# dfyz/osm-renderer

Hardware: AMD Instinct MI355X
Metric: tiles/sec (256x256 z=15) (higher is better)
Workload: dtype f64; 1 GPU; BASELINE.json configs[1]: batch of 1024 z=15 256x256 tiles per GPU, synthetic 50-poly/200-segment geometry per tile (SplitMix64, SURVEY.md 8(d)), lat/lon f64 input resident in HBM, RGBA8 framebuffers written to HBM; 2 batches in flight (step i on resident copy / stream i mod 2: the pre-pass of one batch overlaps the raster stage of the previous one); tiles_this_rank=1024, polygons_per_tile=50, polylines_per_tile=40, scale=1, named_config=True, collective=none (1 GPU), rccl_nranks_seen=1, batches_in_flight=2

## Files before the change

osm_renderer_amd/build.py:

```python
import os
import shutil
import subprocess

HERE = os.path.dirname(os.path.abspath(__file__))
CSRC = os.path.join(HERE, "csrc")
LIB = os.path.join(HERE, "libosmtile.so")
SOURCES = ["osmt_kernels.hip", "osmt_labels.hip", "osmt_glyphs.hip", "osmt_textplace.hip", "osmt_textshape.hip", "osmt_polylabel.hip", "osmt_styled.hip", "osmt_tilequery.hip", "osmt_tilelabels.hip", "osmt_arealabels.hip", "osmt_selmatch.hip", "osmt_labelbind.hip", "osmt_cascade.hip", "osmt_anchors.hip", "osmt_pngenc.hip", "osmt_api.cpp", "osmt_png.cpp"]
HEADERS = ["osmt_bitonic.h", "osmt_cascade_rule.h", "osmt_cascade_tables.h", "osmt_fill_slots.h", "osmt_geom.h", "osmt_glyph.h", "osmt_internal.h", "osmt_list_slices.h", "osmt_numparse.h", "osmt_png_table.h", "osmt_prebin_roles.h", "osmt_project.h", "osmt_utf8.h", os.path.join("..", "host", "osmt_textplacer.hpp"),
           os.path.join("..", "host", "osmt_textshaper.hpp"),
           os.path.join("..", "..", "include", "osmtile.h")]
LIBS = ["-lz", "-ldl", "-lpthread", "-Wl,--no-undefined"]
FLAGS = ["--offload-arch=gfx950", "-O3", "-std=c++17", "-ffp-contract=off", "-fPIC", "-shared", "-Wall"]


def _hipcc():
    for cand in (shutil.which("hipcc"), "/opt/rocm/bin/hipcc"):
        if cand and os.path.exists(cand):
            return cand
    raise RuntimeError("hipcc not found; libosmtile.so cannot be built")


def needs_build():
    if not os.path.exists(LIB):
        return True
    t = os.path.getmtime(LIB)
    deps = [os.path.join(CSRC, s) for s in SOURCES + HEADERS]
    return any(os.path.getmtime(d) > t for d in deps)


def build_variant(name, defines):
    out = os.path.join(HERE, f"libosmtile_{name}.so")
    cmd = [_hipcc()] + FLAGS + [f"-D{d}" for d in defines] + ["-o", out] + [os.path.join(CSRC, s) for s in SOURCES] + LIBS
    subprocess.check_call(cmd)
    return out


def build(force=False, verbose=False):
    if not force and not needs_build():
        return LIB
    cmd = [_hipcc()] + FLAGS + ["-o", LIB] + [os.path.join(CSRC, s) for s in SOURCES] + LIBS
    if verbose:
# ... 8 lines not shown
```

osm_renderer_amd/csrc/osmt_kernels.hip:

```cpp
#include <hip/hip_runtime.h>
#include <stdint.h>

#include "../../include/osmtile.h"
#include "osmt_geom.h"
#include "osmt_internal.h"
#include "osmt_prebin_roles.h"
#include "osmt_project.h"

namespace {

__device__ __forceinline__ uint32_t f64_as_u8(double v) {
#if defined(__HIP_DEVICE_COMPILE__) && !defined(OSMT_V_PLAIN_CVT)
    uint32_t r;
    asm("v_cvt_u32_f64 %0, %1" : "=v"(r) : "v"(v));
    return min(r, 255u);
#else
    return (uint32_t)(int32_t)fmin(fmax(v, 0.0), 255.0);
#endif
}

__device__ __forceinline__ uint32_t wave_incl_scan(uint32_t x) {
    x += (uint32_t)__builtin_amdgcn_update_dpp(0, (int)x, 0x111, 0xF, 0xF, false);
    x += (uint32_t)__builtin_amdgcn_update_dpp(0, (int)x, 0x112, 0xF, 0xF, false);
    x += (uint32_t)__builtin_amdgcn_update_dpp(0, (int)x, 0x114, 0xF, 0xF, false);
    x += (uint32_t)__builtin_amdgcn_update_dpp(0, (int)x, 0x118, 0xF, 0xF, false);
    x += (uint32_t)__builtin_amdgcn_update_dpp(0, (int)x, 0x142, 0xA, 0xF, false);
    x += (uint32_t)__builtin_amdgcn_update_dpp(0, (int)x, 0x143, 0xC, 0xF, false);
    return x;
}

__global__ __launch_bounds__(256) void k_project(const osmt_tile_job* __restrict__ jobs,
                                                 const uint32_t* __restrict__ pt_job,
                                                 const double2* __restrict__ latlon, const uint32_t* __restrict__ refs,
                                                 uint32_t n_pts, double scale, int2* __restrict__ pts, uint32_t* __restrict__ zero,
                                                 uint32_t n_zero) {
    const uint32_t i = blockIdx.x * 256u + threadIdx.x;
    if (i < n_zero) zero[i] = 0u;
    if (i >= n_pts) return;
    const uint32_t j = pt_job[i];
    if (j == 0xFFFFFFFFu) {
// ... 378 lines not shown
            const uint32_t first = q_base + osmt_fill_slot_first(0u, q_incl, nsr);
            const uint32_t g = oi.fill_geom;
            bool past = false;
            for (uint32_t r = 0; r < nsr; ++r) {
                if ((unsigned long long)first + r >= a.slot_cap) {
                    past = true;
                    break;
                }
                a.slots[first + r] = g ? osmt_fill_slot_make(o, oi.arena_off, r, g & 255u, (g >> 8) & 255u, (g >> 16) & 255u, oi.n_rings,
                                                             oi.n_edges, oi.first_pt)
                                       : osmt_fill_slot_empty();
            }
            if (past && a.err) *(volatile uint32_t*)a.err = OSMT_PREPASS_ERR_FILL_ARENA;
        }
    }
    if (live) a.info[o] = oi;
}

__device__ __forceinline__ double opacity_by_center_distance(double cd, double hlw) {
    const double feather_from = fmax(hlw - 0.5, 0.0);
    const double feather_to = fmax(hlw + 0.5, 1.0);
    const double feather_dist = feather_to - feather_from;
    const double opacity_mul = fmin(2.0 * hlw, 1.0);
    double v;
    if (cd < feather_from)
        v = 1.0;
    else if (cd < feather_to)
        v = (feather_to - cd) / feather_dist;
    else
        v = 0.0;
    return opacity_mul * v;
}

#define OSMT_C4(i) (double)(i) / 255.0, (double)((i) + 1) / 255.0, (double)((i) + 2) / 255.0, (double)((i) + 3) / 255.0
#define OSMT_C16(i) OSMT_C4(i), OSMT_C4((i) + 4), OSMT_C4((i) + 8), OSMT_C4((i) + 12)
#define OSMT_C64(i) OSMT_C16(i), OSMT_C16((i) + 16), OSMT_C16((i) + 32), OSMT_C16((i) + 48)
__constant__ double k_u8_over_255[256] = {OSMT_C64(0), OSMT_C64(64), OSMT_C64(128), OSMT_C64(192)};

constexpr int SUB = OSMT_SUB_W;
constexpr int SUBH = OSMT_SUB_H;
constexpr int NTHREADS = 64;
constexpr int PXT = SUB * SUBH / NTHREADS;
constexpr int ROWSTEP = NTHREADS / SUB;
#ifndef OSMT_V_OPCHUNK
#define OSMT_V_OPCHUNK 16
#endif
constexpr int OPCHUNK = OSMT_V_OPCHUNK;
static_assert(OPCHUNK == 16 || OPCHUNK == 32 || OPCHUNK == 64, "a chunk is staged by one wave");
#ifndef OSMT_V_SEGCAP
#define OSMT_V_SEGCAP 32
#endif
constexpr int SEGCAP = OSMT_V_SEGCAP;
static_assert(SEGCAP >= 8 && SEGCAP <= 64, "a filter pass is at most one wave wide");
#ifndef OSMT_V_PLANE_STRIDE
#define OSMT_V_PLANE_STRIDE 32
#endif
constexpr int PLANE_STRIDE = OSMT_V_PLANE_STRIDE;

#if defined(OSMT_ABL) && OSMT_ABL == 5
#define OSMT_DBG(...) __VA_ARGS__
#else
#define OSMT_DBG(...)
#endif
struct alignas(16) StagedEnt {
    double c0, c1, c2;
    double op;
    uint32_t arena;
    uint32_t kind_stage;
    uint32_t aux;
    uint32_t nv;
};
static_assert(sizeof(StagedEnt) == 48, "three 16-byte LDS loads");
struct StrokeConst {
    double ff0, ft0, fd0, rfd0, mul0;
    uint32_t flags;
    uint32_t _pad;
};
constexpr uint32_t STROKE_PLAIN_MAIN = 1u;
constexpr uint32_t STROKE_UNIT_FD = 2u;
constexpr uint32_t STROKE_TINY_MUL = 4u;
constexpr uint32_t STROKE_DASH_FAST = 8u;
__device__ __forceinline__ uint32_t stroke_flags(const osmt_stroke_aux* __restrict__ sa) {
    const bool tiny = !(sa->mul0 >= 1e-100);
    const int n = sa->main_n_segs;
#ifdef OSMT_V_NO_DASH_FAST
    const bool fast = false;
#else
    const bool fast = n > 0 && sa->main_has_orig == 0 && sa->main_total_len > 0.0 && !tiny;
#endif
    return (n == 0 ? STROKE_PLAIN_MAIN : 0u) | (sa->fd0 == 1.0 ? STROKE_UNIT_FD : 0u) | (tiny ? STROKE_TINY_MUL : 0u) | (fast ? STROKE_DASH_FAST : 0u);
}
#ifndef OSMT_V_STAGECAP
#define OSMT_V_STAGECAP 16
#endif
constexpr int STAGECAP = OSMT_V_STAGECAP;

struct alignas(8) SegDer {
    int32_t a, b;
    float r2b, r2a;
    uint32_t w;
    uint32_t n_main;
    double ru, rv;
};
static_assert(sizeof(SegDer) == 40, "five 8-byte LDS words");
constexpr uint32_t SEGW_INCX_NEG = 1u, SEGW_INCY_NEG = 2u, SEGW_SWAP = 4u, SEGW_CAP = 8u, SEGW_SLOW = 16u;

#ifndef OSMT_V_FILTCAP
#define OSMT_V_FILTCAP 256
#endif
constexpr uint32_t FILTCAP = OSMT_V_FILTCAP;
#if OSMT_V_OPCHUNK <= OSMT_V_STAGECAP
#define OSMT_STAGE_UNION 1
#else
#define OSMT_STAGE_UNION 0
#endif
constexpr int DTAB_F = 7;
struct RasterShared {
    OSMT_DBG(uint32_t dbg[12];)
    osmt_srec seg[SEGCAP];
    SegDer der[SEGCAP];
    uint32_t pre[SEGCAP];
    unsigned long long plane[PLANE_STRIDE * SUBH];
    StagedEnt ent[OPCHUNK];
    uint32_t nvi[OPCHUNK];
#if OSMT_STAGE_UNION
    union {
        uint32_t fmask[SUBH];
        StrokeConst sconst;
    } stg[STAGECAP];
#else
    uint32_t fmask_[STAGECAP][SUBH];
    StrokeConst sconst_[STAGECAP];
#endif
    double dtab[OSMT_MAX_DASH_SEGS][DTAB_F];
    uint32_t queue[64];
#ifdef OSMT_V_LDSPAD
    uint8_t occupancy_experiment_pad[OSMT_V_LDSPAD];
#endif
};
#if !(defined(OSMT_ABL) && OSMT_ABL == 5)
static_assert(sizeof(RasterShared) <= 10240, "16 waves per CU (four per SIMD) share 160 KB of LDS");
#endif
#if OSMT_STAGE_UNION
#define SH_FMASK(sh, st) ((sh).stg[st].fmask)
#define SH_SCONST(sh, st) ((sh).stg[st].sconst)
#else
#define SH_FMASK(sh, st) ((sh).fmask_[st])
#define SH_SCONST(sh, st) ((sh).sconst_[st])
// ... 353 lines not shown
                        if (kind == 1u) {
                            const double num = ft0 - cd;
                            const double qv = fd0 == 1.0 ? num : osmt_div_exact(num, fd0, rfd0);
                            const double cdop = mul0 * (cd < ff0 ? 1.0 : qv);
                            atomicMax(&sh.plane[st.ry * PLANE_STRIDE + st.rx], (unsigned long long)__double_as_longlong(initial_opacity * cdop));
                        }
                    } else {
                        slow = true;
                    }
                }
            }
            const unsigned long long sb = __ballot(slow);
            if (sb) {
                const uint32_t ns = (uint32_t)__popcll(sb);
                if (qn + ns > 64u) {
                    dashed_drain(sh, qn, kc, n, total, r_total, initial_opacity, rc);
                    qn = 0u;
                }
                if (slow) sh.queue[qn + (uint32_t)__popcll(sb & ((1ull << fresh_lane()) - 1ull))] = slot_tag | ((uint32_t)st.ry << 5) | (uint32_t)st.rx;
                qn += ns;
            }
            if (active) {
                const bool corr = st.err + st.two_a > st.b;
                dotv += corr ? dot_step + dot_corr : dot_step;
                walk_advance(st);
            }
        }
    }
    if (qn) dashed_drain(sh, qn, kc, n, total, r_total, initial_opacity, rc);
}

template <class Shared>
__device__ __forceinline__ void walk_items(Shared& sh, uint32_t lane, uint32_t slot0, uint32_t nslot, uint32_t item_base, uint32_t it_lo, uint32_t it_hi,
                                           const StrokeConst& kc, uint32_t sflags, const osmt_stroke_aux* __restrict__ sa, double initial_opacity,
                                           const SubRect& rc) {
    OSMT_DBG(if (lane == 0u) { sh.dbg[1] += (it_hi - it_lo + 63u) / 64u; sh.dbg[2] += it_hi - it_lo; })
    const bool main_plain = (sflags & STROKE_PLAIN_MAIN) != 0u;
    const bool unit_fd = (sflags & (STROKE_UNIT_FD | STROKE_TINY_MUL)) == STROKE_UNIT_FD;
    const bool dash_fast = (sflags & STROKE_DASH_FAST) != 0u;
    if (dash_fast) {
        walk_items_dashed(sh, slot0, nslot, item_base, it_lo, it_hi, kc, sa->main_n_segs, sa->main_total_len, sa->main_r_total, initial_opacity, rc);
        const uint32_t l_ = fresh_lane();
        if (!__ballot(l_ < nslot && (sh.der[slot0 + l_].w & SEGW_CAP) != 0u)) return;
    }
    for (uint32_t it = it_lo + lane; it < it_hi; it += 64u) {
        uint32_t lo_s = slot0, n = nslot;
        while (n > 1u) {
            const uint32_t half = n >> 1;
            const bool right = sh.pre[lo_s + half - 1u] <= it;
            lo_s = right ? lo_s + half : lo_s;
            n = right ? n - half : half;
        }
        const uint32_t base_items = (lo_s == slot0) ? item_base : sh.pre[lo_s - 1u];
        const osmt_srec& r = sh.seg[lo_s];
        const SegDer& d = sh.der[lo_s];
        const bool is_cap = (d.w & SEGW_CAP) != 0u;
        RunState st;
        bool skip_first;
        walk_setup(st, r, d, it - base_items, rc, &skip_first);
        if (main_plain && !is_cap) {
            if (unit_fd)
                walk_plain<true>(st, kc, initial_opacity, skip_first, sh.plane);
            else
                walk_plain<false>(st, kc, initial_opacity, skip_first, sh.plane);
        } else {
#ifndef OSMT_V_NODASH
#pragma unroll 1
            for (uint32_t t = main_plain ? 1u : 0u; t < 2u; ++t) {
                if (is_cap != (t == 1u)) continue;
                if (dash_fast && t == 0u) continue;
#ifdef OSMT_V_SKIPHEAVY
                if (t == (OSMT_V_SKIPHEAVY - 1)) continue;
#endif
                const bool cp = t == 1u;
                const osmt_raster_args* la = late_args();
                const osmt_dash_seg* sgs = cp ? &sa->caps_seg : la->dseg + (size_t)(sa - la->aux) * OSMT_MAX_DASH_SEGS;
                walk_dashed(st, kc, cp ? 1 : sa->main_n_segs, (cp ? sa->caps_has_orig : sa->main_has_orig) != 0, cp ? 0.0 : sa->main_total_len,
                            cp ? 0.0 : sa->main_r_total, sgs, sa->half_width, r.traveled, initial_opacity, sh.plane);
            }
#endif
        }
    }
}

__device__ __noinline__ uint32_t fill_row_streaming(const osmt_ring* __restrict__ rings, const int2* __restrict__ pts,
                                                    uint32_t ring_off, uint32_t n_rings, int32_t y, int32_t x0,
                                                    int32_t x1) {
    uint32_t m = 0u;
    int32_t last_x = INT32_MIN;
    int64_t last_e = -1;
    bool have_last = false;
    uint32_t k = 0;
    int32_t from_x = 0;
    for (;;) {
        bool found = false;
        int32_t bx = 0, bxm = 0;
        int64_t be = 0;
        uint32_t eb = 0;
        for (uint32_t r = 0; r < n_rings; ++r) {
            const osmt_ring ring = rings[ring_off + r];
            if (ring.n_pts < 2) continue;
            for (uint32_t e = 0; e + 1 < ring.n_pts; ++e) {
                const int2 p1 = pts[ring.first_pt + e];
                const int2 p2 = pts[ring.first_pt + e + 1];
                int32_t xmn, xmx;
                if (!osmt_fill_row_extent(p1.x, p1.y, p2.x, p2.y, y, &xmn, &xmx)) continue;
                const int64_t ge = (int64_t)eb + e;
                const bool after = !have_last || xmn > last_x || (xmn == last_x && ge > last_e);
                if (!after) continue;
                if (!found || xmn < bx || (xmn == bx && ge < be)) {
                    found = true;
// ... 649 lines not shown
#else
    unsigned long long save;
    double t0, t1, t2, k;
    asm volatile(
        "v_cmp_lt_f64 vcc, 0, %[al]\n\t"
        "s_and_saveexec_b64 %[sv], vcc\n\t"
        "s_cbranch_execz 1f\n\t"
        "v_mul_f64 %[t0], %[al], %[c0]\n\t"
        "v_mul_f64 %[t1], %[al], %[c1]\n\t"
        "v_mul_f64 %[t2], %[al], %[c2]\n\t"
        "v_add_f64 %[k], 1.0, -%[al]\n\t"
        "v_mul_f64 %[r], %[k], %[r]\n\t"
        "v_mul_f64 %[g], %[k], %[g]\n\t"
        "v_mul_f64 %[b], %[k], %[b]\n\t"
        "v_add_f64 %[r], %[t0], %[r]\n\t"
        "v_add_f64 %[g], %[t1], %[g]\n\t"
        "v_add_f64 %[b], %[t2], %[b]\n"
        "1:\n\t"
        "s_mov_b64 exec, %[sv]"
        : [r] "+v"(r), [g] "+v"(g), [b] "+v"(b), [sv] "=&s"(save), [t0] "=&v"(t0), [t1] "=&v"(t1), [t2] "=&v"(t2), [k] "=&v"(k)
        : [al] "v"(al), [c0] "v"(c0), [c1] "v"(c1), [c2] "v"(c2)
        : "vcc", "scc");
#endif
}

template <bool OUT_F64, bool LABELS, bool FOLD>
__global__ OSMT_RASTER_BOUNDS void k_raster(
    const osmt_raster_args a) {
    const osmt_ent* OSMT_R g_ent = a.ent;
    const osmt_stroke_aux* OSMT_R g_aux = a.aux;
    const uint32_t* OSMT_R g_fmask = a.fmask;
    const osmt_srec* OSMT_R g_srec = a.srec;
    const uint2* OSMT_R g_skey = a.skey;
    const uint32_t g_scale = a.scale;
    __shared__ RasterShared sh;

    const uint32_t tid = threadIdx.x;
    const uint32_t lane = tid;
    const uint32_t W = OSMT_TILE_SIZE * g_scale;
    const uint32_t subs_per_row = W / SUB;
    const uint32_t nsub = subs_per_row * (W / SUBH);

    const uint32_t b = blockIdx.x;
    const uint32_t xcd = b & 7u;
    const uint32_t rest = b >> 3;
    const uint32_t tile = (rest / nsub) * 8u + xcd;
    const uint32_t sub = rest % nsub;
    if (tile >= a.n_jobs) return;

    const osmt_tile_job job = a.jobs[tile];
    SubRect rc;
    const uint32_t sub_x = sub % subs_per_row, sub_y = sub / subs_per_row;
    rc.x0 = (int32_t)(sub_x * SUB);
    rc.y0 = (int32_t)(sub_y * SUBH);
    rc.x1 = rc.x0 + SUB - 1;
    rc.y1 = rc.y0 + SUBH - 1;


#ifdef OSMT_V_ACCPROBE
#define AJ(j) ((j) % OSMT_V_ACCPROBE)
#else
#define AJ(j) (j)
#endif
    double acc[PXT][3];
    {
        double r = 0.0, g = 0.0, bl = 0.0;
        if (job.has_canvas) {
            r = 1.0 * k_u8_over_255[job.canvas_rgb[0]];
            g = 1.0 * k_u8_over_255[job.canvas_rgb[1]];
            bl = 1.0 * k_u8_over_255[job.canvas_rgb[2]];
        }
#pragma unroll
        for (int j = 0; j < PXT; ++j) {
            acc[AJ(j)][0] = r;
            acc[AJ(j)][1] = g;
            acc[AJ(j)][2] = bl;
        }
    }
    bool plane_clean = false;
    OSMT_DBG(if (lane < 12) sh.dbg[lane] = 0u; __syncthreads();)

    const bool fold = FOLD && job.n_ops <= OSMT_FOLD_MAX_OPS;
    auto op_bits = [&](unsigned long long* b0, unsigned long long* b1) {
        const osmt_raster_args* la = late_args();
        const osmt_tile_job* OSMT_R jb = &la->jobs[tile];
        const uint32_t n_ops = jb->n_ops, sub_rows = W / SUBH;
        const uint32_t* OSMT_R sm = la->submask + (size_t)jb->op_off * sub_rows + sub / subs_per_row;
        const uint32_t t_ = fresh_lane(), sx_ = sub % subs_per_row;
        const uint32_t w0 = t_ < n_ops ? sm[(size_t)t_ * sub_rows] : 0u;
        const uint32_t w1 = t_ + 64u < n_ops ? sm[(size_t)(t_ + 64u) * sub_rows] : 0u;
        *b0 = __ballot((w0 >> sx_) & 1u);
        *b1 = __ballot((w1 >> sx_) & 1u);
    };
    uint2 hdr = make_uint2(0u, 0u);
    if (fold) {
        unsigned long long b0, b1;
        op_bits(&b0, &b1);
        hdr.y = (uint32_t)__popcll(b0) + (uint32_t)__popcll(b1);
    } else {
        hdr = a.hdr[(size_t)tile * nsub + sub];
        if (job.n_ops == 0u) hdr = make_uint2(0u, 0u);
    }
#if defined(OSMT_ABL) && OSMT_ABL == 8
    const uint32_t n_ent = hdr.y > 0xFFFFFFF0u ? 1u : 0u;
#else
    const uint32_t n_ent = hdr.y;
#endif
    const osmt_ent* OSMT_R my_ent = g_ent + hdr.x;

    for (uint32_t base = 0; base < n_ent; base += OPCHUNK) {
        const uint32_t total = min((uint32_t)OPCHUNK, n_ent - base);
        const bool hit = lane < total;
        osmt_ent e = {};
        if (FOLD && late_args()->jobs[tile].n_ops <= OSMT_FOLD_MAX_OPS) {
            osmt_ent* const tmp = reinterpret_cast<osmt_ent*>(sh.seg);
            static_assert(sizeof(osmt_ent) * OPCHUNK <= sizeof(sh.seg), "a chunk's entries fit the record array");
            const osmt_opinfo* OSMT_R g_info = late_args()->info + late_args()->jobs[tile].op_off;
            unsigned long long bb[2];
            op_bits(&bb[0], &bb[1]);
            const uint32_t n0 = (uint32_t)__popcll(bb[0]);
#pragma unroll
            for (uint32_t half = 0; half < 2u; ++half) {
                const uint32_t t_ = fresh_lane();
                const uint32_t r = (half ? n0 : 0u) + (uint32_t)__popcll(bb[half] & ((1ull << t_) - 1ull));
                if (((bb[half] >> t_) & 1ull) && r >= base && r < base + (uint32_t)OPCHUNK) {
                    const osmt_opinfo* OSMT_R hi = &g_info[t_ + 64u * half];
                    const uint32_t kind = hi->kind;
                    const bool strk = kind == OSMT_OP_STROKE;
                    const uint32_t geom = hi->fill_geom, arena0 = hi->arena_off;
                    osmt_ent t;
                    t.kind_color = kind | ((uint32_t)hi->color[0] << 8) | ((uint32_t)hi->color[1] << 16) | ((uint32_t)hi->color[2] << 24);
                    t.opacity = hi->opacity;
                    t.aux = strk ? hi->aux : hi->image_id;
                    t.nv = strk ? hi->rec_cap : 0u;
                    t.arena = strk ? arena0
                                   : (arena0 + (sub / subs_per_row - (geom & 255u)) * ((geom >> 16) & 255u) + (sub % subs_per_row - ((geom >> 8) & 255u))) * SUBH;
                    t.stage = 0u;
                    t._pad = 0u;
                    tmp[r - base] = t;
                }
            }
            __syncthreads();
            if (hit) e = tmp[fresh_lane()];
        } else if (hit) {
            e = my_ent[base + lane];
        }
        const uint32_t e_kind = e.kind_color & 255u;
        const bool is_stroke = hit && e_kind == OSMT_OP_STROKE;
        const unsigned long long sbal = __ballot(is_stroke);
#if OSMT_STAGE_UNION
        const uint32_t my_stage = fresh_lane();
#else
        const unsigned long long fbal = __ballot(hit && !is_stroke);
        const uint32_t my_stage = (uint32_t)__popcll((is_stroke ? sbal : fbal) & ((1ull << fresh_lane()) - 1ull));
#endif
        const uint32_t nv_scan = wave_incl_scan(is_stroke ? min(e.nv, 1u << 20) : 0u);
        __syncthreads();
        if (hit) {
            sh.nvi[fresh_lane()] = nv_scan;
            StagedEnt se;
            const double cr = k_u8_over_255[(e.kind_color >> 8) & 255u], cg = k_u8_over_255[(e.kind_color >> 16) & 255u],
                         cb = k_u8_over_255[e.kind_color >> 24];
            const bool fc = e_kind == OSMT_OP_FILL_COLOR;
            se.c0 = fc ? e.opacity * cr : cr;
            se.c1 = fc ? e.opacity * cg : cg;
            se.c2 = fc ? e.opacity * cb : cb;
            se.op = fc ? 1.0 - e.opacity : e.opacity;
            se.arena = e.arena;
            se.kind_stage = e_kind | ((my_stage < (uint32_t)STAGECAP ? my_stage : 255u) << 8);
            se.aux = e.aux;
            se.nv = e.nv;
            sh.ent[lane] = se;
            if (!is_stroke && my_stage < (uint32_t)STAGECAP) {
                const uint4* OSMT_R src = reinterpret_cast<const uint4*>(g_fmask + e.arena);
                uint4* dst = reinterpret_cast<uint4*>(&SH_FMASK(sh, my_stage)[0]);
                const uint4 w0 = src[0], w1 = src[1], w2 = src[2], w3 = src[3];
                dst[0] = w0;
                dst[1] = w1;
                dst[2] = w2;
                dst[3] = w3;
            }
            if (is_stroke && my_stage < (uint32_t)STAGECAP) {
                const osmt_stroke_aux* __restrict__ sa = &g_aux[e.aux];
                StrokeConst kc;
                kc.ff0 = sa->ff0;
                kc.ft0 = sa->ft0;
                kc.fd0 = sa->fd0;
                kc.rfd0 = sa->rfd0;
                kc.mul0 = sa->mul0;
                kc.flags = stroke_flags(sa);
                kc._pad = 0;
                SH_SCONST(sh, my_stage) = kc;
            }
        }
        const bool any_stroke = sbal != 0ull;
        if (any_stroke && !plane_clean) {
            static_assert((PLANE_STRIDE * SUBH) % NTHREADS == 0, "the plane is cleared in whole wave strides");
            const uint32_t t_ = fresh_lane();
#pragma unroll
            for (uint32_t i = 0; i < PLANE_STRIDE * SUBH; i += NTHREADS) sh.plane[i + t_] = 0ull;
            plane_clean = true;
        }
        __syncthreads();

        uint32_t g0 = 0;
#if defined(OSMT_ABL) && OSMT_ABL == 7
        if (total < 1000u) g0 = total;
#endif
        while (g0 < total) {
        uint32_t gend = total, V = 0;
        bool big = false;
        uint32_t s_before = 0u;
        const uint32_t nv_incl = any_stroke ? sh.nvi[fresh_lane() & (uint32_t)(OPCHUNK - 1)] : 0u;
        if (any_stroke) {
            s_before = g0 ? (uint32_t)__builtin_amdgcn_readlane((int)nv_incl, (int)g0 - 1) : 0u;
            const unsigned long long over = __ballot(lane >= g0 && lane < total && nv_incl - s_before > (uint32_t)FILTCAP);
            if (over) gend = (uint32_t)__builtin_ctzll(over);
            if (gend == g0) {
                OSMT_DBG(if (lane == 0) sh.dbg[7] += 1u;)
                big = true;
                gend = g0 + 1u;
            } else {
                V = (uint32_t)__builtin_amdgcn_readlane((int)nv_incl, (int)gend - 1) - s_before;
            }
        }
        if (V) {
// ... 109 lines not shown
            }
            __syncthreads();
        }
        unsigned long long gbal = 0ull;

        for (uint32_t li = g0; li < gend; ++li) {
            const StagedEnt& en = sh.ent[li];
            const uint32_t ks = (uint32_t)__builtin_amdgcn_readfirstlane((int)en.kind_stage);
            const uint32_t kind = ks & 255u, stage = ks >> 8;
            const double cop = en.op;
#if defined(OSMT_ABL) && OSMT_ABL == 6
            if (kind != 77u) continue;
#endif
#if defined(OSMT_ABL) && OSMT_ABL == 3
            if (kind == OSMT_OP_STROKE) continue;
#endif
#if defined(OSMT_ABL) && OSMT_ABL == 4
            if (kind != OSMT_OP_STROKE) continue;
#endif
            if (kind == OSMT_OP_STROKE) {
                OSMT_DBG(if (lane == 0) sh.dbg[0] += 1u;)
                const uint32_t aux_i = (uint32_t)__builtin_amdgcn_readfirstlane((int)en.aux);
                const osmt_stroke_aux* __restrict__ sa = &g_aux[aux_i];
                StrokeConst kc;
                if (stage != 255u) {
                    kc = SH_SCONST(sh, stage);
                } else {
                    kc.ff0 = sa->ff0;
                    kc.ft0 = sa->ft0;
                    kc.fd0 = sa->fd0;
                    kc.rfd0 = sa->rfd0;
                    kc.mul0 = sa->mul0;
                    kc.flags = stroke_flags(sa);
                    kc._pad = 0;
                }
                const uint32_t sflags = (uint32_t)__builtin_amdgcn_readfirstlane((int)kc.flags);
                if (sflags & STROKE_DASH_FAST) {
                    const double* OSMT_R src = reinterpret_cast<const double*>(late_args()->dseg + (size_t)aux_i * OSMT_MAX_DASH_SEGS);
                    static_assert(sizeof(osmt_dash_seg) == 9 * sizeof(double), "nine doubles per DashSegment");
                    const uint32_t nd = (uint32_t)sa->main_n_segs * (uint32_t)DTAB_F;
                    for (uint32_t l = fresh_lane(); l < nd; l += 64u) {
                        const uint32_t sg = l / (uint32_t)DTAB_F, f = l % (uint32_t)DTAB_F;
                        (&sh.dtab[0][0])[l] = src[sg * 9u + (f < 5u ? f : f + 2u)];
                    }
                    __syncthreads();
                }
                uint32_t n_rounds = 1u, big_cap = 0u, arena = 0u;
                if (big) {
                    big_cap = (uint32_t)__builtin_amdgcn_readfirstlane((int)en.nv);
                    arena = (uint32_t)__builtin_amdgcn_readfirstlane((int)en.arena);
                    n_rounds = (big_cap + (uint32_t)SEGCAP - 1u) / (uint32_t)SEGCAP;
                }
                for (uint32_t round = 0; round < n_rounds; ++round) {
                    uint32_t slot0 = 0u, nslot = 0u;
                    if (big) {
                        __syncthreads();
                        uint32_t ridx = 0xFFFFFFFFu;
                        const uint32_t v = round * (uint32_t)SEGCAP + lane;
                        if (lane < (uint32_t)SEGCAP && v < big_cap) ridx = arena + v;
                        uint32_t cnt = 0, is_cap = 0;
                        if (ridx != 0xFFFFFFFFu) {
                            const uint2 key = g_skey[ridx];
                            if (key.x == sub) {
                                cnt = key.y & 0x7FFFFFFFu;
                                is_cap = key.y >> 31;
                            }
                        }
                        gbal = __ballot(cnt > 0u);
                        const uint32_t incl = wave_incl_scan(cnt);
                        if (cnt > 0u) {
                            const uint32_t slot = (uint32_t)__popcll(gbal & ((1ull << fresh_lane()) - 1ull));
                            const osmt_srec r = g_srec[ridx];
                            sh.seg[slot] = r;
                            sh.der[slot] = seg_derive(r, is_cap != 0u);
                            sh.pre[slot] = incl;
                        }
                        __syncthreads();
                        nslot = (uint32_t)__popcll(gbal);
                    } else {
                        slot0 = (uint32_t)__builtin_amdgcn_readfirstlane((int)en.arena);
                        nslot = (uint32_t)__builtin_amdgcn_readfirstlane((int)en.nv);
                    }
                    {
                        if (nslot) {
                            const uint32_t item_lo = slot0 ? (uint32_t)__builtin_amdgcn_readfirstlane((int)sh.pre[slot0 - 1u]) : 0u;
                            const uint32_t item_hi = (uint32_t)__builtin_amdgcn_readfirstlane((int)sh.pre[slot0 + nslot - 1u]);
#if defined(OSMT_ABL) && (OSMT_ABL == 1 || OSMT_ABL == 2)
                            (void)item_lo; (void)item_hi;
#else
                            walk_items(sh, lane, slot0, nslot, item_lo, item_lo, item_hi, kc, sflags, sa, cop, rc);
#endif
                        }
                    }
                }
                __syncthreads();
#if defined(OSMT_ABL) && OSMT_ABL == 2
                if (false)
#endif
                {
                    const StagedEnt& eb = sh.ent[late_index(li)];
                    const double c0 = eb.c0, c1 = eb.c1, c2 = eb.c2;
                    const uint32_t t_ = fresh_lane();
                    const uint32_t cell0 = (t_ / SUB) * PLANE_STRIDE + (t_ & (SUB - 1));
#pragma unroll
                    for (int j = 0; j < PXT; ++j) {
                        const uint32_t idx = cell0 + (uint32_t)j * ROWSTEP * PLANE_STRIDE;
                        const double al = __longlong_as_double((long long)sh.plane[idx]);
                        sh.plane[idx] = 0ull;
                        blend_stroke_masked(acc[AJ(j)][0], acc[AJ(j)][1], acc[AJ(j)][2], al, c0, c1, c2);
                    }
                }
                __syncthreads();
            }
            if (late_index(kind) != OSMT_OP_STROKE) {
                OSMT_DBG(if (lane == 0) sh.dbg[5] += 1u;)
                uint32_t w_[SUBH];
                if (stage != 255u) {
                    const uint4* OSMT_R lw = reinterpret_cast<const uint4*>(&SH_FMASK(sh, stage)[0]);
#pragma unroll
                    for (int q = 0; q < SUBH / 4; ++q) {
                        const uint4 v = lw[q];
                        w_[4 * q + 0] = v.x;
                        w_[4 * q + 1] = v.y;
// ... 95 lines not shown
            }
          }
        }
    }

    void* const g_out = late_args()->out;
    const size_t g_out_tile_stride = late_args()->out_tile_stride;
    const uint32_t t_out = fresh_lane();
    const uint32_t lx_o = t_out & (SUB - 1), ly_o = t_out / SUB;
    if (!OUT_F64 && late_args()->out_rgb8) {
        uint8_t* const stg = reinterpret_cast<uint8_t*>(sh.plane);
        static_assert(sizeof(sh.plane) >= (size_t)SUB * SUBH * 3, "RGB8 staging fits the alpha plane");
        __syncthreads();
#pragma unroll
        for (int j = 0; j < PXT; ++j) {
            const uint32_t row = ly_o + (uint32_t)j * ROWSTEP;
            uint8_t* px = stg + (row * SUB + lx_o) * 3u;
            px[0] = (uint8_t)f64_as_u8(255.0 * acc[AJ(j)][0]);
            px[1] = (uint8_t)f64_as_u8(255.0 * acc[AJ(j)][1]);
            px[2] = (uint8_t)f64_as_u8(255.0 * acc[AJ(j)][2]);
        }
        __syncthreads();
        constexpr uint32_t ROW_DW = SUB * 3 / 4;
        uint8_t* const tile_out = reinterpret_cast<uint8_t*>(g_out) + (size_t)tile * g_out_tile_stride;
#pragma unroll
        for (uint32_t q = 0; q < ROW_DW * SUBH / NTHREADS; ++q) {
            const uint32_t d = q * NTHREADS + t_out;
            const uint32_t row = d / ROW_DW, k = d % ROW_DW;
            const uint32_t v = reinterpret_cast<const uint32_t*>(stg)[d];
            __builtin_nontemporal_store(v, reinterpret_cast<uint32_t*>(tile_out + ((size_t)(rc.y0 + (int32_t)row) * W + (size_t)rc.x0) * 3u + 4u * k));
        }
        return;
    }
#pragma unroll
    for (int j = 0; j < PXT; ++j) {
        const uint32_t row = ly_o + (uint32_t)j * ROWSTEP;
        const size_t px = (size_t)(rc.y0 + (int32_t)row) * W + (size_t)(rc.x0 + (int32_t)lx_o);
        if (OUT_F64) {
            double4* out = reinterpret_cast<double4*>(g_out) + (size_t)tile * W * W + px;
            *out = make_double4(acc[AJ(j)][0], acc[AJ(j)][1], acc[AJ(j)][2], 1.0);
        } else {
            const uint32_t v = f64_as_u8(255.0 * acc[AJ(j)][0]) | (f64_as_u8(255.0 * acc[AJ(j)][1]) << 8) |
                               (f64_as_u8(255.0 * acc[AJ(j)][2]) << 16) | 0xFF000000u;
            uint32_t* out = reinterpret_cast<uint32_t*>(reinterpret_cast<uint8_t*>(g_out) +
                                                        (size_t)tile * g_out_tile_stride) + px;
#ifdef OSMT_V_PLAIN_STORE
            *out = v;
#else
            __builtin_nontemporal_store(v, out);
#endif
            OSMT_DBG(__syncthreads(); if (j == 0 && ly_o == 0 && lx_o < 12) *out = sh.dbg[lx_o];)
        }
    }
}

typedef double v2d __attribute__((ext_vector_type(2)));

__device__ __forceinline__ double dpp_swap_pair(double x) {
    const long long b = __double_as_longlong(x);
    const int lo = __builtin_amdgcn_update_dpp(0, (int)(b & 0xFFFFFFFFll), 0xB1, 0xF, 0xF, false);
    const int hi = __builtin_amdgcn_update_dpp(0, (int)(b >> 32), 0xB1, 0xF, 0xF, false);
    return __longlong_as_double(((long long)hi << 32) | (unsigned int)lo);
}

template <int LT, bool NT>
__global__ __launch_bounds__(256) void k_composite(const v2d* __restrict__ planes, double4 canvas, uint32_t n,
// ... 201 lines not shown
```

Before: 1.488 million tiles/s.

## Shorten raster kernel dependency chains at start, staging, dash visit and store

Several small latency-chain reductions in the raster kernel. Job and header records are now loaded with explicit scalar loads, and the canvas colour is computed arithmetically instead of through a constant-memory table lookup. Entry staging issues the fill-mask and stroke-aux loads early as vector words and builds the stroke constants from them, with the dash main-segment fields cached in LDS so walk_items no longer reads global aux. The RGBA8 store path uses precomputed byte offsets. Each piece is gated by a macro; the inline asm and layout static_asserts add fragility.

New measurement: 1.553 million tiles/s (median of 6 runs). 4.3% higher.

```diff
diff --git a/osm_renderer_amd/build.py b/osm_renderer_amd/build.py
--- a/osm_renderer_amd/build.py
+++ b/osm_renderer_amd/build.py
@@ -6,7 +6,7 @@
 CSRC = os.path.join(HERE, "csrc")
 LIB = os.path.join(HERE, "libosmtile.so")
 SOURCES = ["osmt_kernels.hip", "osmt_labels.hip", "osmt_glyphs.hip", "osmt_textplace.hip", "osmt_textshape.hip", "osmt_polylabel.hip", "osmt_styled.hip", "osmt_tilequery.hip", "osmt_tilelabels.hip", "osmt_arealabels.hip", "osmt_selmatch.hip", "osmt_labelbind.hip", "osmt_cascade.hip", "osmt_anchors.hip", "osmt_pngenc.hip", "osmt_api.cpp", "osmt_png.cpp"]
-HEADERS = ["osmt_bitonic.h", "osmt_cascade_rule.h", "osmt_cascade_tables.h", "osmt_fill_slots.h", "osmt_geom.h", "osmt_glyph.h", "osmt_internal.h", "osmt_list_slices.h", "osmt_numparse.h", "osmt_png_table.h", "osmt_prebin_roles.h", "osmt_project.h", "osmt_utf8.h", os.path.join("..", "host", "osmt_textplacer.hpp"),
+HEADERS = ["osmt_bitonic.h", "osmt_cascade_rule.h", "osmt_cascade_tables.h", "osmt_fill_slots.h", "osmt_geom.h", "osmt_glyph.h", "osmt_internal.h", "osmt_list_slices.h", "osmt_numparse.h", "osmt_png_table.h", "osmt_prebin_roles.h", "osmt_project.h", "osmt_u8_over_255.h", "osmt_utf8.h", os.path.join("..", "host", "osmt_textplacer.hpp"),
            os.path.join("..", "host", "osmt_textshaper.hpp"),
            os.path.join("..", "..", "include", "osmtile.h")]
 LIBS = ["-lz", "-ldl", "-lpthread", "-Wl,--no-undefined"]
diff --git a/osm_renderer_amd/csrc/osmt_kernels.hip b/osm_renderer_amd/csrc/osmt_kernels.hip
--- a/osm_renderer_amd/csrc/osmt_kernels.hip
+++ b/osm_renderer_amd/csrc/osmt_kernels.hip
@@ -6,6 +6,7 @@
 #include "osmt_internal.h"
 #include "osmt_prebin_roles.h"
 #include "osmt_project.h"
+#include "osmt_u8_over_255.h"
 
 namespace {
 
@@ -450,19 +451,39 @@
     return opacity_mul * v;
 }
 
-#define OSMT_C4(i) (double)(i) / 255.0, (double)((i) + 1) / 255.0, (double)((i) + 2) / 255.0, (double)((i) + 3) / 255.0
-#define OSMT_C16(i) OSMT_C4(i), OSMT_C4((i) + 4), OSMT_C4((i) + 8), OSMT_C4((i) + 12)
-#define OSMT_C64(i) OSMT_C16(i), OSMT_C16((i) + 16), OSMT_C16((i) + 32), OSMT_C16((i) + 48)
-__constant__ double k_u8_over_255[256] = {OSMT_C64(0), OSMT_C64(64), OSMT_C64(128), OSMT_C64(192)};
 
 constexpr int SUB = OSMT_SUB_W;
 constexpr int SUBH = OSMT_SUB_H;
 constexpr int NTHREADS = 64;
 constexpr int PXT = SUB * SUBH / NTHREADS;
 constexpr int ROWSTEP = NTHREADS / SUB;
+#ifndef OSMT_V_CHAIN_START
+#define OSMT_V_CHAIN_START 1
+#endif
+#ifndef OSMT_V_CHAIN_COLOR
+#define OSMT_V_CHAIN_COLOR 1
+#endif
+#ifndef OSMT_V_CHAIN_STAGE
+#define OSMT_V_CHAIN_STAGE 1
+#endif
+#ifndef OSMT_V_CHAIN_VISIT
+#define OSMT_V_CHAIN_VISIT 1
+#endif
+#ifndef OSMT_V_CHAIN_STORE
+#define OSMT_V_CHAIN_STORE 1
+#endif
 #ifndef OSMT_V_OPCHUNK
 #define OSMT_V_OPCHUNK 16
 #endif
+#ifndef OSMT_V_STAGECAP
+#define OSMT_V_STAGECAP 16
+#endif
+#if OSMT_V_OPCHUNK <= OSMT_V_STAGECAP
+#define OSMT_STAGE_UNION 1
+#else
+#define OSMT_STAGE_UNION 0
+#endif
+#define OSMT_CHAIN_VISIT (OSMT_V_CHAIN_VISIT && OSMT_STAGE_UNION)
 constexpr int OPCHUNK = OSMT_V_OPCHUNK;
 static_assert(OPCHUNK == 16 || OPCHUNK == 32 || OPCHUNK == 64, "a chunk is staged by one wave");
 #ifndef OSMT_V_SEGCAP
@@ -492,8 +513,18 @@
 struct StrokeConst {
     double ff0, ft0, fd0, rfd0, mul0;
     uint32_t flags;
+#if OSMT_CHAIN_VISIT
+    uint32_t n_segs;
+    double total_len, r_total;
+#else
     uint32_t _pad;
+#endif
 };
+#if OSMT_CHAIN_VISIT
+#define OSMT_KC_MAIN(sh, stage, sa, f, m) (SH_SCONST(sh, late_index(stage)).f)
+#else
+#define OSMT_KC_MAIN(sh, stage, sa, f, m) ((sa)->m)
+#endif
 constexpr uint32_t STROKE_PLAIN_MAIN = 1u;
 constexpr uint32_t STROKE_UNIT_FD = 2u;
 constexpr uint32_t STROKE_TINY_MUL = 4u;
@@ -508,9 +539,6 @@
 #endif
     return (n == 0 ? STROKE_PLAIN_MAIN : 0u) | (sa->fd0 == 1.0 ? STROKE_UNIT_FD : 0u) | (tiny ? STROKE_TINY_MUL : 0u) | (fast ? STROKE_DASH_FAST : 0u);
 }
-#ifndef OSMT_V_STAGECAP
-#define OSMT_V_STAGECAP 16
-#endif
 constexpr int STAGECAP = OSMT_V_STAGECAP;
 
 struct alignas(8) SegDer {
@@ -527,11 +555,6 @@
 #define OSMT_V_FILTCAP 256
 #endif
 constexpr uint32_t FILTCAP = OSMT_V_FILTCAP;
-#if OSMT_V_OPCHUNK <= OSMT_V_STAGECAP
-#define OSMT_STAGE_UNION 1
-#else
-#define OSMT_STAGE_UNION 0
-#endif
 constexpr int DTAB_F = 7;
 struct RasterShared {
     OSMT_DBG(uint32_t dbg[12];)
@@ -951,14 +974,15 @@
 
 template <class Shared>
 __device__ __forceinline__ void walk_items(Shared& sh, uint32_t lane, uint32_t slot0, uint32_t nslot, uint32_t item_base, uint32_t it_lo, uint32_t it_hi,
-                                           const StrokeConst& kc, uint32_t sflags, const osmt_stroke_aux* __restrict__ sa, double initial_opacity,
-                                           const SubRect& rc) {
+                                           const StrokeConst& kc, uint32_t stage, uint32_t sflags, const osmt_stroke_aux* __restrict__ sa,
+                                           double initial_opacity, const SubRect& rc) {
     OSMT_DBG(if (lane == 0u) { sh.dbg[1] += (it_hi - it_lo + 63u) / 64u; sh.dbg[2] += it_hi - it_lo; })
     const bool main_plain = (sflags & STROKE_PLAIN_MAIN) != 0u;
     const bool unit_fd = (sflags & (STROKE_UNIT_FD | STROKE_TINY_MUL)) == STROKE_UNIT_FD;
     const bool dash_fast = (sflags & STROKE_DASH_FAST) != 0u;
     if (dash_fast) {
-        walk_items_dashed(sh, slot0, nslot, item_base, it_lo, it_hi, kc, sa->main_n_segs, sa->main_total_len, sa->main_r_total, initial_opacity, rc);
+        walk_items_dashed(sh, slot0, nslot, item_base, it_lo, it_hi, kc, OSMT_KC_MAIN(sh, stage, sa, n_segs, main_n_segs), OSMT_KC_MAIN(sh, stage, sa, total_len, main_total_len),
+                          OSMT_KC_MAIN(sh, stage, sa, r_total, main_r_total), initial_opacity, rc);
         const uint32_t l_ = fresh_lane();
         if (!__ballot(l_ < nslot && (sh.der[slot0 + l_].w & SEGW_CAP) != 0u)) return;
     }
@@ -994,8 +1018,8 @@
                 const bool cp = t == 1u;
                 const osmt_raster_args* la = late_args();
                 const osmt_dash_seg* sgs = cp ? &sa->caps_seg : la->dseg + (size_t)(sa - la->aux) * OSMT_MAX_DASH_SEGS;
-                walk_dashed(st, kc, cp ? 1 : sa->main_n_segs, (cp ? sa->caps_has_orig : sa->main_has_orig) != 0, cp ? 0.0 : sa->main_total_len,
-                            cp ? 0.0 : sa->main_r_total, sgs, sa->half_width, r.traveled, initial_opacity, sh.plane);
+                walk_dashed(st, kc, cp ? 1 : (int)OSMT_KC_MAIN(sh, stage, sa, n_segs, main_n_segs), (cp ? sa->caps_has_orig : sa->main_has_orig) != 0,
+                            cp ? 0.0 : OSMT_KC_MAIN(sh, stage, sa, total_len, main_total_len), cp ? 0.0 : OSMT_KC_MAIN(sh, stage, sa, r_total, main_r_total), sgs, sa->half_width, r.traveled, initial_opacity, sh.plane);
             }
 #endif
         }
@@ -1711,7 +1735,15 @@
     const uint32_t* OSMT_R g_fmask = a.fmask;
     const osmt_srec* OSMT_R g_srec = a.srec;
     const uint2* OSMT_R g_skey = a.skey;
+#if OSMT_V_CHAIN_START
+    const osmt_tile_job* OSMT_R g_jobs = a.jobs;
+    const uint2* OSMT_R g_hdr = a.hdr;
+    uint32_t g_n_jobs = a.n_jobs;
+    uint32_t g_scale = a.scale;
+    asm("" : "+s"(g_n_jobs), "+s"(g_scale) : "s"(g_jobs), "s"(g_hdr), "s"(g_ent), "s"(g_aux), "s"(g_fmask), "s"(g_srec), "s"(g_skey));
+#else
     const uint32_t g_scale = a.scale;
+#endif
     __shared__ RasterShared sh;
 
     const uint32_t tid = threadIdx.x;
@@ -1725,9 +1757,39 @@
     const uint32_t rest = b >> 3;
     const uint32_t tile = (rest / nsub) * 8u + xcd;
     const uint32_t sub = rest % nsub;
+#if OSMT_V_CHAIN_START
+    if (tile >= g_n_jobs) return;
+
+    struct alignas(32) JobWords {
+        uint32_t w[8];
+    };
+    static_assert(sizeof(osmt_tile_job) == sizeof(JobWords) && offsetof(osmt_tile_job, has_canvas) == 9 && offsetof(osmt_tile_job, canvas_rgb) == 10 &&
+                      offsetof(osmt_tile_job, n_ops) == 16 && offsetof(osmt_tile_job, op_off) == 20,
+                  "the job record as words");
+    uint32_t job_w2, job_w3, job_n_ops;
+    uint2 hdr_raw = make_uint2(0u, 0u);
+    if (FOLD) {
+        const JobWords jw = *reinterpret_cast<const JobWords*>(g_jobs + tile);
+        job_w2 = jw.w[2], job_w3 = jw.w[3], job_n_ops = jw.w[4];
+    } else {
+        typedef uint32_t u32x4 __attribute__((ext_vector_type(4)));
+        typedef uint32_t u32x2 __attribute__((ext_vector_type(2)));
+        u32x4 jq;
+        u32x2 hq;
+        asm("s_load_dwordx4 %0, %2, 0x8\n\t"
+            "s_load_dwordx2 %1, %3, 0x0\n\t"
+            "s_waitcnt lgkmcnt(0)"
+            : "=&s"(jq), "=&s"(hq)
+            : "s"(g_jobs + tile), "s"(g_hdr + ((size_t)tile * nsub + sub)));
+        job_w2 = jq.x, job_w3 = jq.y, job_n_ops = jq.z;
+        hdr_raw = make_uint2(hq.x, hq.y);
+    }
+#else
     if (tile >= a.n_jobs) return;
 
     const osmt_tile_job job = a.jobs[tile];
+    const uint32_t job_n_ops = job.n_ops;
+#endif
     SubRect rc;
     const uint32_t sub_x = sub % subs_per_row, sub_y = sub / subs_per_row;
     rc.x0 = (int32_t)(sub_x * SUB);
@@ -1744,11 +1806,24 @@
     double acc[PXT][3];
     {
         double r = 0.0, g = 0.0, bl = 0.0;
+#if OSMT_V_CHAIN_START
+        const bool has_canvas = ((job_w2 >> 8) & 255u) != 0u;
+        auto uniform = [](double v) {
+            const long long b = __double_as_longlong(v);
+            const uint32_t lo = (uint32_t)__builtin_amdgcn_readfirstlane((int)(b & 0xFFFFFFFFll));
+            const uint32_t hi = (uint32_t)__builtin_amdgcn_readfirstlane((int)(b >> 32));
+            return __longlong_as_double((long long)(((unsigned long long)hi << 32) | lo));
+        };
+        r = uniform(osmt_u8_over_255(has_canvas ? (job_w2 >> 16) & 255u : 0u));
+        g = uniform(osmt_u8_over_255(has_canvas ? job_w2 >> 24 : 0u));
+        bl = uniform(osmt_u8_over_255(has_canvas ? job_w3 & 255u : 0u));
+#else
         if (job.has_canvas) {
             r = 1.0 * k_u8_over_255[job.canvas_rgb[0]];
             g = 1.0 * k_u8_over_255[job.canvas_rgb[1]];
             bl = 1.0 * k_u8_over_255[job.canvas_rgb[2]];
         }
+#endif
 #pragma unroll
         for (int j = 0; j < PXT; ++j) {
             acc[AJ(j)][0] = r;
@@ -1759,7 +1834,7 @@
     bool plane_clean = false;
     OSMT_DBG(if (lane < 12) sh.dbg[lane] = 0u; __syncthreads();)
 
-    const bool fold = FOLD && job.n_ops <= OSMT_FOLD_MAX_OPS;
+    const bool fold = FOLD && job_n_ops <= OSMT_FOLD_MAX_OPS;
     auto op_bits = [&](unsigned long long* b0, unsigned long long* b1) {
         const osmt_raster_args* la = late_args();
         const osmt_tile_job* OSMT_R jb = &la->jobs[tile];
@@ -1777,8 +1852,12 @@
         op_bits(&b0, &b1);
         hdr.y = (uint32_t)__popcll(b0) + (uint32_t)__popcll(b1);
     } else {
+#if OSMT_V_CHAIN_START
+        hdr = FOLD ? a.hdr[(size_t)tile * nsub + sub] : hdr_raw;
+#else
         hdr = a.hdr[(size_t)tile * nsub + sub];
-        if (job.n_ops == 0u) hdr = make_uint2(0u, 0u);
+#endif
+        if (job_n_ops == 0u) hdr = make_uint2(0u, 0u);
     }
 #if defined(OSMT_ABL) && OSMT_ABL == 8
     const uint32_t n_ent = hdr.y > 0xFFFFFFF0u ? 1u : 0u;
@@ -1837,9 +1916,18 @@
         __syncthreads();
         if (hit) {
             sh.nvi[fresh_lane()] = nv_scan;
+#if OSMT_V_CHAIN_STAGE && OSMT_STAGE_UNION
+            const uint4* OSMT_R src = is_stroke ? reinterpret_cast<const uint4*>(&g_aux[e.aux]) + 1 : reinterpret_cast<const uint4*>(g_fmask + e.arena);
+            const uint4 w0 = src[0], w1 = src[1], w2 = src[2], w3 = src[3];
+#endif
             StagedEnt se;
+#if OSMT_V_CHAIN_COLOR
+            const double cr = osmt_u8_over_255((e.kind_color >> 8) & 255u), cg = osmt_u8_over_255((e.kind_color >> 16) & 255u),
+                         cb = osmt_u8_over_255(e.kind_color >> 24);
+#else
             const double cr = k_u8_over_255[(e.kind_color >> 8) & 255u], cg = k_u8_over_255[(e.kind_color >> 16) & 255u],
                          cb = k_u8_over_255[e.kind_color >> 24];
+#endif
             const bool fc = e_kind == OSMT_OP_FILL_COLOR;
             se.c0 = fc ? e.opacity * cr : cr;
             se.c1 = fc ? e.opacity * cg : cg;
@@ -1850,6 +1938,42 @@
             se.aux = e.aux;
             se.nv = e.nv;
             sh.ent[lane] = se;
+#if OSMT_V_CHAIN_STAGE && OSMT_STAGE_UNION
+            {
+                static_assert(offsetof(osmt_stroke_aux, ff0) == 16 && offsetof(osmt_stroke_aux, ft0) == 24 && offsetof(osmt_stroke_aux, fd0) == 32 &&
+                                  offsetof(osmt_stroke_aux, mul0) == 40 && offsetof(osmt_stroke_aux, rfd0) == 48 &&
+                                  offsetof(osmt_stroke_aux, main_n_segs) == 56 && offsetof(osmt_stroke_aux, main_has_orig) == 60 &&
+                                  offsetof(osmt_stroke_aux, main_total_len) == 64 && offsetof(osmt_stroke_aux, main_r_total) == 72 &&
+                                  sizeof(StrokeConst) == (OSMT_CHAIN_VISIT ? 64 : 48) && sizeof(uint32_t) * SUBH == 64,
+                              "the words the stroke constants are put together from");
+                uint4* dst = reinterpret_cast<uint4*>(&SH_FMASK(sh, my_stage)[0]);
+                dst[0] = w0;
+                if (is_stroke) {
+                    auto f64_of = [](uint32_t lo, uint32_t hi) { return __longlong_as_double((long long)(((unsigned long long)hi << 32) | lo)); };
+                    const double fd0 = f64_of(w1.x, w1.y), mul0 = f64_of(w1.z, w1.w), total_len = f64_of(w3.x, w3.y);
+                    const int n = (int)w2.z;
+                    const bool tiny = !(mul0 >= 1e-100);
+#ifdef OSMT_V_NO_DASH_FAST
+                    const bool fast = false;
+#else
+                    const bool fast = n > 0 && w2.w == 0u && total_len > 0.0 && !tiny;
+#endif
+                    const uint32_t flags =
+                        (n == 0 ? STROKE_PLAIN_MAIN : 0u) | (fd0 == 1.0 ? STROKE_UNIT_FD : 0u) | (tiny ? STROKE_TINY_MUL : 0u) | (fast ? STROKE_DASH_FAST : 0u);
+                    dst[1] = make_uint4(w1.x, w1.y, w2.x, w2.y);
+#if OSMT_CHAIN_VISIT
+                    dst[2] = make_uint4(w1.z, w1.w, flags, w2.z);
+                    dst[3] = w3;
+#else
+                    dst[2] = make_uint4(w1.z, w1.w, flags, 0u);
+#endif
+                } else {
+                    dst[1] = w1;
+                    dst[2] = w2;
+                    dst[3] = w3;
+                }
+            }
+#else
             if (!is_stroke && my_stage < (uint32_t)STAGECAP) {
                 const uint4* OSMT_R src = reinterpret_cast<const uint4*>(g_fmask + e.arena);
                 uint4* dst = reinterpret_cast<uint4*>(&SH_FMASK(sh, my_stage)[0]);
@@ -1868,9 +1992,16 @@
                 kc.rfd0 = sa->rfd0;
                 kc.mul0 = sa->mul0;
                 kc.flags = stroke_flags(sa);
+#if OSMT_CHAIN_VISIT
+                kc.n_segs = (uint32_t)sa->main_n_segs;
+                kc.total_len = sa->main_total_len;
+                kc.r_total = sa->main_r_total;
+#else
                 kc._pad = 0;
+#endif
                 SH_SCONST(sh, my_stage) = kc;
             }
+#endif
         }
         const bool any_stroke = sbal != 0ull;
         if (any_stroke && !plane_clean) {
@@ -2046,13 +2177,19 @@
                     kc.rfd0 = sa->rfd0;
                     kc.mul0 = sa->mul0;
                     kc.flags = stroke_flags(sa);
+#if OSMT_CHAIN_VISIT
+                    kc.n_segs = (uint32_t)sa->main_n_segs;
+                    kc.total_len = sa->main_total_len;
+                    kc.r_total = sa->main_r_total;
+#else
                     kc._pad = 0;
+#endif
                 }
                 const uint32_t sflags = (uint32_t)__builtin_amdgcn_readfirstlane((int)kc.flags);
                 if (sflags & STROKE_DASH_FAST) {
                     const double* OSMT_R src = reinterpret_cast<const double*>(late_args()->dseg + (size_t)aux_i * OSMT_MAX_DASH_SEGS);
                     static_assert(sizeof(osmt_dash_seg) == 9 * sizeof(double), "nine doubles per DashSegment");
-                    const uint32_t nd = (uint32_t)sa->main_n_segs * (uint32_t)DTAB_F;
+                    const uint32_t nd = (uint32_t)OSMT_KC_MAIN(sh, stage, sa, n_segs, main_n_segs) * (uint32_t)DTAB_F;
                     for (uint32_t l = fresh_lane(); l < nd; l += 64u) {
                         const uint32_t sg = l / (uint32_t)DTAB_F, f = l % (uint32_t)DTAB_F;
                         (&sh.dtab[0][0])[l] = src[sg * 9u + (f < 5u ? f : f + 2u)];
@@ -2102,7 +2239,7 @@
 #if defined(OSMT_ABL) && (OSMT_ABL == 1 || OSMT_ABL == 2)
                             (void)item_lo; (void)item_hi;
 #else
-                            walk_items(sh, lane, slot0, nslot, item_lo, item_lo, item_hi, kc, sflags, sa, cop, rc);
+                            walk_items(sh, lane, slot0, nslot, item_lo, item_lo, item_hi, kc, stage, sflags, sa, cop, rc);
 #endif
                         }
                     }
@@ -2264,6 +2401,20 @@
         }
         return;
     }
+#if OSMT_V_CHAIN_STORE
+    if (!OUT_F64) {
+        typedef __attribute__((address_space(1))) uint32_t global_u32;
+        uint8_t* const sub_out = reinterpret_cast<uint8_t*>(g_out) + (size_t)tile * g_out_tile_stride + ((size_t)rc.y0 * W + (size_t)rc.x0) * 4u;
+        const uint32_t off0 = (ly_o * W + lx_o) * 4u, row_step = (uint32_t)ROWSTEP * W * 4u;
+#pragma unroll
+        for (int j = 0; j < PXT; ++j) {
+            const uint32_t v = f64_as_u8(255.0 * acc[AJ(j)][0]) | (f64_as_u8(255.0 * acc[AJ(j)][1]) << 8) |
+                               (f64_as_u8(255.0 * acc[AJ(j)][2]) << 16) | 0xFF000000u;
+            __builtin_nontemporal_store(v, (global_u32*)(sub_out + (off0 + (uint32_t)j * row_step)));
+        }
+        return;
+    }
+#endif
 #pragma unroll
     for (int j = 0; j < PXT; ++j) {
         const uint32_t row = ly_o + (uint32_t)j * ROWSTEP;
diff --git a/osm_renderer_amd/csrc/osmt_u8_over_255.h b/osm_renderer_amd/csrc/osmt_u8_over_255.h
--- /dev/null
+++ b/osm_renderer_amd/csrc/osmt_u8_over_255.h
@@ -0,0 +1,20 @@
+#ifndef OSMT_U8_OVER_255_H
+#define OSMT_U8_OVER_255_H
+
+#include <stdint.h>
+
+#include "osmt_geom.h"
+
+#define OSMT_C4(i) (double)(i) / 255.0, (double)((i) + 1) / 255.0, (double)((i) + 2) / 255.0, (double)((i) + 3) / 255.0
+#define OSMT_C16(i) OSMT_C4(i), OSMT_C4((i) + 4), OSMT_C4((i) + 8), OSMT_C4((i) + 12)
+#define OSMT_C64(i) OSMT_C16(i), OSMT_C16((i) + 16), OSMT_C16((i) + 32), OSMT_C16((i) + 48)
+#if defined(__HIPCC__)
+static __constant__
+#else
+static const
+#endif
+    double k_u8_over_255[256] = {OSMT_C64(0), OSMT_C64(64), OSMT_C64(128), OSMT_C64(192)};
+
+OSMT_HD double osmt_u8_over_255(uint32_t c) { return osmt_div_exact((double)c, 255.0, 1.0 / 255.0); }
+
+#endif
```
